# cvYouTian/Dedark-YOLO

Hardware: AMD Instinct MI355X
Metric: training img/s at 640x640 (higher is better)
Workload: dtype bf16

## Files before the change

### dedark_yolo_amd/csrc/conv_v5.hip

```cpp
#include <stdlib.h>
#include <type_traits>
#include "dy_common.h"
#include "conv_epilogue.h"
#include "../../include/dedark_yolo.h"

namespace v5 {

constexpr int BM = 256, BK = 32;
constexpr int A_BYTES = BM * 64, NSTAGE = 3;
constexpr unsigned B_ROW_OOB = 0x40000000u;

typedef __attribute__((address_space(3))) void* lds_ptr_t;
typedef __attribute__((ext_vector_type(8))) __bf16 bf16x8;

__device__ unsigned long long g_stamps[16];

__device__ inline void stamp(int ablate, int nblk, int i) {
  if ((ablate & 32) && threadIdx.x == 0 && (blockIdx.x == 0 || (int)blockIdx.x == (nblk / 8) * 7)) {
    unsigned long long t;
    asm volatile("s_memtime %0\n\ts_waitcnt lgkmcnt(0)" : "=s"(t)::"memory");
    g_stamps[(blockIdx.x == 0 ? 0 : 8) + i] = t;
  }
}

struct P {
  const char* src;
  const char* w;
  char* dst;
  unsigned src_bytes, w_bytes;
  long src_ld, dst_ld, dst_row, dst_img;
  int Hs, Ws, Cs, Hd, Wd, Cd;
  int stride;
  int KH, KW;
  int dh0, dhs, dw0, dws;
  int kh0, khs, kw0, kws, KWf;
  long w_row;
  const float* scale;
  const float* shift;
  int act;
  double* stats;
  int accumulate;
  long M;
  int a_min;
  int nk;
  int tiles_n, nblk;
  const char* add_src;
  long add_src_ld;
  int ablate;
  int ncls;
  DyParityCls cls[4];
};

__device__ inline int xcd_remap(int bid, int nblk) {
  int q = nblk >> 3, r = nblk & 7, x = bid & 7;
  int base = (x < r) ? x * (q + 1) : r * (q + 1) + (x - r) * q;
  return base + (bid >> 3);
}

__device__ inline long dst_offset(const P& p, long m) {
  if (p.dst_row == 0) return m * p.dst_ld;
  const long HWd = (long)p.Hd * p.Wd;
  const long img = m / HWd;
  const int rem = (int)(m - img * HWd);
  const int oh = rem / p.Wd, ow = rem - oh * p.Wd;
  return img * p.dst_img + (long)oh * p.dst_row + (long)ow * p.dst_ld;
}

template <int BN, typename T, int MB>
__device__ __forceinline__ void epilogue(const P& p, f32x4 (&acc)[MB][4], char* smem, int tid, int lane, int wave, int wm, int wn, long m0,
                                         int n0, int tile_m) {
  constexpr int WN = BN / 64, WM = 4 / WN;
  constexpr int PT = dy_epi::row_pitch<BN>();
  const int cl = lane & 15, g = lane >> 4;
  const bool plain = !p.scale && !p.shift && p.act == DY_ACT_NONE;
#pragma unroll
  for (int j = 0; j < 4; ++j) {
    const int c0 = 64 * wn + 16 * j + 4 * g;
    if (plain) {
#pragma unroll
      for (int i = 0; i < MB; ++i) {
        const int px = 16 * MB * wm + 16 * i + cl;
        uint2 w2 = {dy_epi::pack2<T>(acc[i][j][0], acc[i][j][1]), dy_epi::pack2<T>(acc[i][j][2], acc[i][j][3])};
        *reinterpret_cast<uint2*>(smem + px * PT + c0 * 2) = w2;
      }
    } else {
      float sc[4], sf[4];
#pragma unroll
      for (int e = 0; e < 4; ++e) {
        const int n = n0 + c0 + e;
        const bool nok = n < p.Cd;
        sc[e] = (nok && p.scale) ? p.scale[n] : 1.f;
        sf[e] = (nok && p.shift) ? p.shift[n] : 0.f;
      }
#pragma unroll
      for (int i = 0; i < MB; ++i) {
        const int px = 16 * MB * wm + 16 * i + cl;
        float v[4];
#pragma unroll
        for (int e = 0; e < 4; ++e) {
          float u = acc[i][j][e] * sc[e] + sf[e];
          if (p.act == DY_ACT_SILU) u = u * dy_sigmoid(u);
          else if (p.act == DY_ACT_LEAKY) u = u > 0.f ? u : 0.1f * u;
          v[e] = u;
        }
        uint2 w2 = {dy_epi::pack2<T>(v[0], v[1]), dy_epi::pack2<T>(v[2], v[3])};
        *reinterpret_cast<uint2*>(smem + px * PT + c0 * 2) = w2;
      }
    }
  }
  __syncthreads();
  stamp(DY_ABLATE_OF(p), p.nblk, 3);
  dy_epi::store_rows<BM, BN, 4>(smem, lane, wave, m0, n0, p.M, p.Cd, p.accumulate, reinterpret_cast<T*>(p.dst),
                                [&](long m) { return dst_offset(p, m); }, reinterpret_cast<const T*>(p.add_src), p.add_src_ld);
  stamp(DY_ABLATE_OF(p), p.nblk, 4);
  if (p.stats) {
    __syncthreads();
    float* red = reinterpret_cast<float*>(smem);
#pragma unroll
    for (int j = 0; j < 4; ++j)
#pragma unroll
      for (int e = 0; e < 4; ++e) {
        float s1 = 0.f, s2 = 0.f;
#pragma unroll
        for (int i = 0; i < MB; ++i) {
          const float a = acc[i][j][e];
          s1 += a;
          s2 += a * a;
        }
        s1 = row16_sum(s1);
        s2 = row16_sum(s2);
        if (cl == 0) {
          const int col = 64 * wn + 16 * j + 4 * g + e;
          red[(wm * BN + col) * 2] = s1;
          red[(wm * BN + col) * 2 + 1] = s2;
        }
      }
    __syncthreads();
    if (tid < BN) {
      const int n = n0 + tid;
      if (n < p.Cd) {
        float s1 = 0.f, s2 = 0.f;
#pragma unroll
        for (int w = 0; w < WM; ++w) {
          s1 += red[(w * BN + tid) * 2];
          s2 += red[(w * BN + tid) * 2 + 1];
        }
        double* st = p.stats + (long)(tile_m % DY_STATS_REPLICAS) * 2 * p.Cd;
        atomic_add_f64(st + n, (double)s1);
        atomic_add_f64(st + p.Cd + n, (double)s2);
      }
    }
  }
}

template <int BN, typename T = bf16_t, bool SLIM = false>
__global__ __launch_bounds__(256, SLIM ? 4 : 2) void conv_kernel(const P pk) {
  constexpr int WN = BN / 64, WM = 4 / WN, MB = BM / WM / 16, NB = 4, STAGE = A_BYTES + BN * 64, B_LD = BN / 64;
  extern __shared__ __attribute__((aligned(16))) char smem[];
  const int tid = threadIdx.x, lane = tid & 63;
  const int wave = __builtin_amdgcn_readfirstlane(tid >> 6);
  const int wm = wave / WN, wn = wave % WN;
  P p = pk;
  int bid;
  if (pk.ncls > 1) {
    const int x = blockIdx.x & 7, i = (int)blockIdx.x >> 3;
    int c = 0;
#pragma unroll
    for (int k = 1; k < 4; ++k)
      if (k < pk.ncls && i >= pk.cls[k].blk0) c = k;
    const DyParityCls& k = pk.cls[c];
    bid = x * k._r + (i - k.blk0);
    if (bid >= (int)((k.M + BM - 1) / BM) * pk.tiles_n) return;
    p.dst = k.dst; p.M = k.M; p.Hd = k.Hd; p.Wd = k.Wd; p.KH = k.KH; p.KW = k.KW;
    p.dh0 = -k.pad; p.dw0 = -k.pad; p.kh0 = k.kh0; p.kw0 = k.kw0;
    p.nk = k.Ktot / BK;
    p.a_min = -(k.pad * pk.Ws + k.pad) * (int)pk.src_ld * 2;
  } else {
    bid = xcd_remap(blockIdx.x, p.nblk);
  }
  stamp(DY_ABLATE_OF(p), p.nblk, 0);
  const int tile_m = bid / p.tiles_n, tile_n = bid - tile_m * p.tiles_n;
  const long m0 = (long)tile_m * BM;
  const int n0 = tile_n * BN;

  unsigned nrec_a = p.nk > 0 ? p.src_bytes - p.a_min : 0, nrec_b = p.nk > 0 ? p.w_bytes : 0;

  const int lrow = lane >> 2, slot = lane & 3;
  const int chunk = slot ^ ((lane & 32) ? 3 : 0);
  unsigned a_off[4], a_pad[4], b_off[B_LD];
  {
    const DyTileWalk walk(m0, p.Hd, p.Wd);
#pragma unroll
    for (int j = 0; j < 4; ++j) {
      const int r = 16 * (wave + 4 * j) + lrow;
      const bool ok = m0 + r < p.M;
      int img, oh, ow;
      walk.at(r, img, oh, ow);
      const int sh0 = oh * p.stride, sw0 = ow * p.stride;
      a_off[j] = (unsigned)((((long)img * p.Hs + sh0) * p.Ws + sw0) * p.src_ld * 2 + chunk * 16);
      unsigned wb = 0, mk = 0;
      for (int tw = 0; tw < p.KW; ++tw) {
        const int sw = sw0 + p.dw0 + p.dws * tw;
        if (sw >= 0 && sw < p.Ws) wb |= 1u << tw;
      }
      for (int th = 0; th < p.KH; ++th) {
        const int sh = sh0 + p.dh0 + p.dhs * th;
        if (ok && sh >= 0 && sh < p.Hs) mk |= wb << (th * p.KW);
      }
      if (DY_ABLATE_OF(p) & 2) mk = 0;
      else if (DY_ABLATE_OF(p) & 1) mk &= 1u;
      a_pad[j] = __builtin_amdgcn_alignbit(~mk, ~mk, 1);
    }
#pragma unroll
    for (int j = 0; j < B_LD; ++j) {
      const int n = n0 + 16 * (wave + 4 * j) + lrow;
      b_off[j] = (n < p.Cd && !(DY_ABLATE_OF(p) & 4)) ? (unsigned)((long)n * p.w_row * 2 + chunk * 16) : B_ROW_OOB;
    }
  }
  const int ntaps = p.KH * p.KW;
  int vtap_a, vtap_b;
  {
    const int t = lane < ntaps ? lane : 0;
    const int th = t / p.KW, tw = t - th * p.KW;
    vtap_a = ((p.dh0 + p.dhs * th) * p.Ws + p.dw0 + p.dws * tw) * (int)p.src_ld * 2 - p.a_min;
    vtap_b = (int)((((long)((p.kh0 + p.khs * th) * p.KWf + p.kw0 + p.kws * tw)) * p.Cs) * 2);
  }
  int sk = 0, s_tap = 0, s_ci2 = 0;
  int a_koff = __builtin_amdgcn_readlane(vtap_a, 0), b_koff = __builtin_amdgcn_readlane(vtap_b, 0);
  auto advance = [&]() {
    ++sk;
    const bool wrap = s_tap + 1 == ntaps;
    s_tap = wrap ? 0 : s_tap + 1;
    s_ci2 += wrap ? 2 * BK : 0;
    a_koff = __builtin_amdgcn_readlane(vtap_a, s_tap) + s_ci2;
    b_koff = __builtin_amdgcn_readlane(vtap_b, s_tap) + s_ci2;
    const int rot = wrap ? (33 - ntaps) & 31 : 1;
#pragma unroll
    for (int j = 0; j < 4; ++j) a_pad[j] = __builtin_amdgcn_alignbit(a_pad[j], a_pad[j], rot);
    if (sk >= p.nk) { nrec_a = 0; nrec_b = 0; a_koff = 0; b_koff = 0; }
  };
  auto issue = [&](int base) {
    const __amdgpu_buffer_rsrc_t rs_a = __builtin_amdgcn_make_buffer_rsrc((void*)(p.src + p.a_min), 0, nrec_a, 0x00020000);
    const __amdgpu_buffer_rsrc_t rs_b = __builtin_amdgcn_make_buffer_rsrc((void*)p.w, 0, nrec_b, 0x00020000);
#pragma unroll
    for (int j = 0; j < 4; ++j) {
      if ((DY_ABLATE_OF(p) & 64) && s_tap) continue;
      const unsigned v = (a_pad[j] & 0x80000000u) | a_off[j];
      __builtin_amdgcn_raw_ptr_buffer_load_lds(rs_a, (lds_ptr_t)(smem + base + (wave + 4 * j) * 1024), 16, (int)v, a_koff, 0, 0);
    }
#pragma unroll
    for (int j = 0; j < B_LD; ++j)
      __builtin_amdgcn_raw_ptr_buffer_load_lds(rs_b, (lds_ptr_t)(smem + base + A_BYTES + (wave + 4 * j) * 1024), 16, (int)b_off[j], b_koff, 0,
                                               0);
  };

  const int fr = lane & 15, fq = lane >> 4;
  const int sw = (fq ^ ((fr & 8) ? 3 : 0)) * 16;
  const int a_rd = (16 * MB * wm + fr) * 64 + sw;
  const int b_rd = A_BYTES + (64 * wn + fr) * 64 + sw;

  f32x4 acc[MB][NB];
#pragma unroll
  for (int i = 0; i < MB; ++i)
#pragma unroll
    for (int j = 0; j < 4; ++j) acc[i][j] = f32x4{0.f, 0.f, 0.f, 0.f};

  auto compute = [&](int base, auto mid) {
    u32x4 bfr[NB], afr[MB];
    if (DY_ABLATE_OF(p) & 16) {
#pragma unroll
      for (int j = 0; j < 4; ++j) bfr[j] = u32x4{0x3f803f80u + (unsigned)base, 0x3f803f80u, 0x3f803f80u, 0x3f803f80u};
#pragma unroll
      for (int i = 0; i < MB; ++i) afr[i] = u32x4{0x3f803f80u, 0x3f803f80u + (unsigned)lane, 0x3f803f80u, 0x3f803f80u};
    } else {
#pragma unroll
      for (int j = 0; j < 4; ++j) bfr[j] = *reinterpret_cast<const u32x4*>(smem + base + b_rd + 1024 * j);
#pragma unroll
      for (int i = 0; i < MB; ++i) afr[i] = *reinterpret_cast<const u32x4*>(smem + base + a_rd + 1024 * i);
    }
    if (DY_ABLATE_OF(p) & 8) {
#pragma unroll
      for (int i = 0; i < MB; ++i) acc[i][0][0] += __builtin_bit_cast(float, afr[i][0] ^ bfr[i & 3][1]);
      mid();
      return;
    }
    __builtin_amdgcn_s_setprio(1);
#pragma unroll
    for (int i = 0; i < MB; ++i) {
#pragma unroll
      for (int j = 0; j < NB; ++j)
        acc[i][j] = mfma_16x16x32<T>(bfr[j], afr[i], acc[i][j]);
      if (i == 0) mid();
    }
    __builtin_amdgcn_s_setprio(0);
  };
  auto nothing = []() {};
  auto walk = [&]() { advance(); };
  stamp(DY_ABLATE_OF(p), p.nblk, 1);
  if constexpr (BN >= 128) {
    issue(0);
    advance();
    issue(STAGE);
    advance();
    int cur = 0, fill = 2 * STAGE;
    for (int kt = 0; kt < p.nk; ++kt) {
      if ((DY_ABLATE_OF(p) & 64) || kt + 1 >= p.nk) asm volatile("s_waitcnt vmcnt(0)" ::: "memory");
      else
      asm volatile("s_waitcnt vmcnt(%0)" ::"n"(4 + B_LD) : "memory");
      __builtin_amdgcn_s_barrier();
      __builtin_amdgcn_sched_barrier(0);
      if (sk < p.nk) issue(fill);
      __builtin_amdgcn_sched_barrier(0);
      compute(cur, walk);
      __builtin_amdgcn_sched_barrier(0);
      cur = cur == 2 * STAGE ? 0 : cur + STAGE;
      fill = fill == 2 * STAGE ? 0 : fill + STAGE;
    }
  } else if constexpr (SLIM) {
    issue(0);
    advance();
    int cur = 0;
    for (int kt = 0; kt < p.nk; ++kt) {
      asm volatile("s_waitcnt vmcnt(0)" ::: "memory");
      __builtin_amdgcn_s_barrier();
      __builtin_amdgcn_sched_barrier(0);
      if (sk < p.nk) issue(cur ? 0 : STAGE);
      __builtin_amdgcn_sched_barrier(0);
      compute(cur, walk);
      __builtin_amdgcn_sched_barrier(0);
      cur = cur ? 0 : STAGE;
    }
  } else {
    issue(0);
    advance();
    issue(STAGE);
    advance();
    int cur = 0;
    for (int kt = 0; kt < p.nk; kt += 2) {
      asm volatile("s_waitcnt vmcnt(0)" ::: "memory");
      __builtin_amdgcn_s_barrier();
      __builtin_amdgcn_sched_barrier(0);
      const int nxt = cur ^ (2 * STAGE);
      if (sk < p.nk) {
        issue(nxt);
        advance();
        issue(nxt + STAGE);
      } else {
        advance();
      }
      __builtin_amdgcn_sched_barrier(0);
      compute(cur, walk);
      compute(cur + STAGE, nothing);
      __builtin_amdgcn_sched_barrier(0);
      cur = nxt;
    }
  }
  asm volatile("s_waitcnt vmcnt(0)" ::: "memory");
  __builtin_amdgcn_s_barrier();
  stamp(DY_ABLATE_OF(p), p.nblk, 2);

  epilogue<BN, T, MB>(p, acc, smem, tid, lane, wave, wm, wn, m0, n0, tile_m);
#ifdef DY_DIAG
  asm volatile("s_waitcnt vmcnt(0)" ::: "memory");
#endif
  stamp(DY_ABLATE_OF(p), p.nblk, 5);
}

constexpr int BAND_BYTES = 17 * 1024;

template <int BN, typename T = bf16_t, int NBAND_ = (BN == 64 ? 3 : 2)>
__global__ __launch_bounds__(256, (BN == 64 && NBAND_ == 2) ? 3 : 2) void band_kernel(const P p) {
  constexpr int WN = BN / 64, WM = 4 / WN, MB = BM / WM / 16, B_LD = BN / 64, B_BYTES = BN * 64;
  constexpr int NBAND = NBAND_, DB = 3 * (NBAND - 1), NBBUF = DB + 1;
  constexpr int OFF_B = NBAND * BAND_BYTES, OFF_ZERO = OFF_B + NBBUF * B_BYTES;
  constexpr int N0 = (DB - 1) * B_LD + 5 * (NBAND - 2), N1 = (DB - 1) * B_LD + 5 * (NBAND - 1);
  extern __shared__ __attribute__((aligned(16))) char smem[];
  const int tid = threadIdx.x, lane = tid & 63;
  const int wave = __builtin_amdgcn_readfirstlane(tid >> 6);
  const int wm = wave / WN, wn = wave % WN;
  const int bid = xcd_remap(blockIdx.x, p.nblk);
  stamp(DY_ABLATE_OF(p), p.nblk, 0);
  const int tile_m = bid / p.tiles_n, tile_n = bid - tile_m * p.tiles_n;
  const long m0 = (long)tile_m * BM;
  const int n0 = tile_n * BN;

  if (tid < 16) reinterpret_cast<unsigned*>(smem + OFF_ZERO)[tid] = 0u;

  const int lrow = lane >> 2, slot = lane & 3;
  const int chunk = slot ^ ((lane & 16) ? 2 : 0);
  const bool tail_lane = (lane >> 4) == wave;
  unsigned a_off[5], b_off[B_LD];
#pragma unroll
  for (int j = 0; j < 5; ++j) {
    const int brow = j < 4 ? 16 * (wave + 4 * j) + lrow : 256 + lrow;
    a_off[j] = (unsigned)((m0 - 1 + brow) * p.src_ld * 2 + chunk * 16);
  }
#pragma unroll
  for (int j = 0; j < B_LD; ++j) {
    const int n = n0 + 16 * (wave + 4 * j) + lrow;
    b_off[j] = n < p.Cd ? (unsigned)((long)n * p.w_row * 2 + chunk * 16) : B_ROW_OOB;
  }
  const int ng = p.nk / 3;
  int ga_n = 0, ga_th = 0, ga_ci = 0;
  auto issue_band = [&](int base) {
    const bool live = ga_n < ng && !(DY_ABLATE_OF(p) & 2);
    const unsigned koff = (unsigned)((p.dh0 + p.dhs * ga_th) * p.Ws * (int)p.src_ld * 2 + ga_ci * 2);
    const __amdgpu_buffer_rsrc_t rs = __builtin_amdgcn_make_buffer_rsrc((void*)p.src, 0, live ? p.src_bytes : 0u, 0x00020000);
#pragma unroll
    for (int j = 0; j < 4; ++j)
      __builtin_amdgcn_raw_ptr_buffer_load_lds(rs, (lds_ptr_t)(smem + base + (wave + 4 * j) * 1024), 16, (int)(a_off[j] + koff), 0, 0, 0);
    if (tail_lane)
      __builtin_amdgcn_raw_ptr_buffer_load_lds(rs, (lds_ptr_t)(smem + base + 16 * 1024), 16, (int)(a_off[4] + koff), 0, 0, 0);
    ++ga_n;
    if (++ga_th == 3) { ga_th = 0; ga_ci += BK; }
  };
  int kb = 0, kb_tp = 0, kb_ci = 0;
  auto issue_b = [&](int base) {
    const bool live = kb < p.nk && !(DY_ABLATE_OF(p) & 4);
    const int koff = live ? (int)(((long)kb_tp * p.Cs + kb_ci) * 2) : 0;
    const __amdgpu_buffer_rsrc_t rs = __builtin_amdgcn_make_buffer_rsrc((void*)p.w, 0, live ? p.w_bytes : 0u, 0x00020000);
#pragma unroll
    for (int j = 0; j < B_LD; ++j)
      __builtin_amdgcn_raw_ptr_buffer_load_lds(rs, (lds_ptr_t)(smem + base + (wave + 4 * j) * 1024), 16, (int)b_off[j], koff, 0, 0);
    ++kb;
    if (++kb_tp == 9) { kb_tp = 0; kb_ci += BK; }
  };

  const int fr = lane & 15, fq = lane >> 4;
  const int r0 = 16 * MB * wm + fr;
  int a_rd[3];
#pragma unroll
  for (int tw = 0; tw < 3; ++tw) {
    const int brow = r0 + 1 + p.dw0 + p.dws * tw;
    a_rd[tw] = brow * 64 + ((fq ^ ((brow & 4) ? 2 : 0)) * 16);
  }
  const int b_rd = (64 * wn + fr) * 64 + ((fq ^ ((fr & 4) ? 2 : 0)) * 16);
  unsigned tm[3] = {0u, 0u, 0u};
  {
    const long m = m0 + r0;
    int img, h, w;
    DyTileWalk(m0, p.Hd, p.Wd).at(r0, img, h, w);
#pragma unroll
    for (int i = 0; i < MB; ++i) {
      const bool ok = m + 16 * i < p.M;
#pragma unroll
      for (int th = 0; th < 3; ++th) {
        const bool hv = (unsigned)(h + p.dh0 + p.dhs * th) < (unsigned)p.Hs;
#pragma unroll
        for (int tw = 0; tw < 3; ++tw) {
          const bool wv = (unsigned)(w + p.dw0 + p.dws * tw) < (unsigned)p.Ws;
          if (ok && hv && wv) tm[th] |= 1u << (8 * tw + i);
        }
      }
      w += 16;
      if (w >= p.Wd) {
        w -= p.Wd;
        if (++h == p.Hd) h = 0;
      }
    }
  }

  f32x4 acc[MB][4];
#pragma unroll
  for (int i = 0; i < MB; ++i)
#pragma unroll
    for (int j = 0; j < 4; ++j) acc[i][j] = f32x4{0.f, 0.f, 0.f, 0.f};

  auto compute = [&](int band_base, int b_base, unsigned bits, int ard) {
    u32x4 bfr[4], afr[MB];
    const int av = band_base + ard;
    if (DY_ABLATE_OF(p) & 16) {
#pragma unroll
      for (int j = 0; j < 4; ++j) bfr[j] = u32x4{0x3f803f80u + (unsigned)b_base, 0x3f803f80u, 0x3f803f80u, 0x3f803f80u};
#pragma unroll
      for (int i = 0; i < MB; ++i) afr[i] = u32x4{0x3f803f80u, 0x3f803f80u + (bits & 1u), 0x3f803f80u, 0x3f803f80u};
    } else {
#pragma unroll
      for (int j = 0; j < 4; ++j) bfr[j] = *reinterpret_cast<const u32x4*>(smem + b_base + b_rd + 1024 * j);
#pragma unroll
      for (int i = 0; i < MB; ++i) {
        const int sel = ((bits >> i) & 1u) ? av : OFF_ZERO - 1024 * i;
        afr[i] = *reinterpret_cast<const u32x4*>(smem + sel + 1024 * i);
      }
    }
    if (DY_ABLATE_OF(p) & 8) {
#pragma unroll
      for (int i = 0; i < MB; ++i) acc[i][0][0] += __builtin_bit_cast(float, afr[i][0] ^ bfr[i & 3][1]);
      return;
    }
    __builtin_amdgcn_s_setprio(1);
#pragma unroll
    for (int i = 0; i < MB; ++i)
#pragma unroll
      for (int j = 0; j < 4; ++j) acc[i][j] = mfma_16x16x32<T>(bfr[j], afr[i], acc[i][j]);
    __builtin_amdgcn_s_setprio(0);
  };
  stamp(DY_ABLATE_OF(p), p.nblk, 1);

  int band_fill = 0, b_fill = 0;
#pragma unroll
  for (int s = 0; s < DB; ++s) {
    if (s % 3 == 0) {
      issue_band(band_fill);
      band_fill += BAND_BYTES;
    }
    issue_b(OFF_B + b_fill);
    b_fill += B_BYTES;
  }
  int band_cur = 0, b_cur = 0, th = 0;
  auto next_b = [&]() {
    b_cur = b_cur == DB * B_BYTES ? 0 : b_cur + B_BYTES;
    b_fill = b_fill == DB * B_BYTES ? 0 : b_fill + B_BYTES;
  };
  auto group = [&](auto tailc) {
    constexpr bool tail = decltype(tailc)::value;
    const unsigned tmc = th == 0 ? tm[0] : (th == 1 ? tm[1] : tm[2]);
    asm volatile("s_waitcnt vmcnt(%0)" ::"n"(N0) : "memory");
    __builtin_amdgcn_s_barrier();
    __builtin_amdgcn_sched_barrier(0);
    if constexpr (!tail) {
      issue_band(band_fill);
      issue_b(OFF_B + b_fill);
    }
    __builtin_amdgcn_sched_barrier(0);
    compute(band_cur, OFF_B + b_cur, tmc, a_rd[0]);
    __builtin_amdgcn_sched_barrier(0);
    next_b();
    asm volatile("s_waitcnt vmcnt(%0)" ::"n"(tail ? B_LD : N1) : "memory");
    __builtin_amdgcn_s_barrier();
    __builtin_amdgcn_sched_barrier(0);
    if constexpr (!tail) issue_b(OFF_B + b_fill);
    __builtin_amdgcn_sched_barrier(0);
    compute(band_cur, OFF_B + b_cur, tmc >> 8, a_rd[1]);
    __builtin_amdgcn_sched_barrier(0);
    next_b();
    asm volatile("s_waitcnt vmcnt(%0)" ::"n"(tail ? 0 : N1) : "memory");
    __builtin_amdgcn_s_barrier();
    __builtin_amdgcn_sched_barrier(0);
    if constexpr (!tail) issue_b(OFF_B + b_fill);
    __builtin_amdgcn_sched_barrier(0);
    compute(band_cur, OFF_B + b_cur, tmc >> 16, a_rd[2]);
    __builtin_amdgcn_sched_barrier(0);
    next_b();
    band_cur = band_cur == (NBAND - 1) * BAND_BYTES ? 0 : band_cur + BAND_BYTES;
    band_fill = band_fill == (NBAND - 1) * BAND_BYTES ? 0 : band_fill + BAND_BYTES;
    th = th == 2 ? 0 : th + 1;
  };
  constexpr bool peel = NBAND == 2;
  for (int g = 0; g < ng - (peel ? 1 : 0); ++g) group(std::false_type{});
  if (peel) group(std::true_type{});
  asm volatile("s_waitcnt vmcnt(0)" ::: "memory");
  __builtin_amdgcn_s_barrier();
  stamp(DY_ABLATE_OF(p), p.nblk, 2);
  epilogue<BN, T, MB>(p, acc, smem, tid, lane, wave, wm, wn, m0, n0, tile_m);
#ifdef DY_DIAG
  asm volatile("s_waitcnt vmcnt(0)" ::: "memory");
#endif
  stamp(DY_ABLATE_OF(p), p.nblk, 5);
}


}

extern "C" int dy_debug_conv5_stamps(unsigned long long* out) {
  return hipMemcpyFromSymbol(out, HIP_SYMBOL(v5::g_stamps), sizeof(unsigned long long) * 16) == hipSuccess ? 0 : 1;
}

bool dy_conv_v5_eligible(const dy_conv_desc* d, int mode) {
  static const bool off = dy_env("DY_NO_CONV_V5") != nullptr;
  if (off || (d->dtype != DY_BF16 && d->dtype != DY_F16)) return false;
  if (!(d->Cs % 32 == 0 && d->KH * d->KW <= 25)) return false;
  if (mode == 1 && d->stride != 1) return false;
  if ((d->src_ld * 2) % 16 != 0 || (d->dst_ld * 2) % 16 != 0 || ((uintptr_t)d->dst) % 16 != 0) return false;
  const long M = (long)d->N * d->Hd * d->Wd;
  const long src_bytes = (((long)d->N * d->Hs * d->Ws - 1) * d->src_ld + d->Cs) * 2;
  const long w_row = d->KHf > 0 ? (long)d->KHf * d->KWf * d->Cs : (long)d->KH * d->KW * d->Cs;
  const long w_bytes = (long)d->Cd * w_row * 2;
  const long halo = ((long)d->KH * d->dil * d->Ws + (long)d->KW * d->dil) * d->src_ld * 2;
  if (!(src_bytes + halo <= 0x7fffffffL && w_bytes <= 0x3fffffffL && M < (1L << 31))) return false;
  const long tiles_m = (M + 255) / 256;
  const long tn = (d->Cd + 127) / 128;
  if (d->Cd >= 96 && tn * 128 * 4 <= (long)d->Cd * 5 && tiles_m * tn >= 256) return true;
  return d->Cd >= 48 && d->Cd <= 64 && tiles_m >= 256;
}

static int v5_launch(const dy_conv_desc* d, int mode, void* stream, const dy_conv_desc* classes, int ncls);

int dy_conv_v5_launch(const dy_conv_desc* d, int mode, void* stream) { return v5_launch(d, mode, stream, nullptr, 0); }

bool dy_conv_v5_classes_eligible(const dy_conv_desc* c, int ncls) {
  static const bool off = dy_env("DY_NO_CONV_V5") != nullptr || (dy_env("DY_V5_CLASSES") && atoi(dy_env("DY_V5_CLASSES")) == 0);
  if (off || ncls < 2 || ncls > 4) return false;
  const dy_conv_desc* d = &c[0];
  if (d->dtype != DY_BF16 && d->dtype != DY_F16) return false;
  if (!(d->Cs % 32 == 0 && d->KHf > 0 && d->KHf * d->KWf <= 25 && d->stride == 1)) return false;
  const long src_bytes = (((long)d->N * d->Hs * d->Ws - 1) * d->src_ld + d->Cs) * 2;
  const long w_bytes = (long)d->Cd * d->KHf * d->KWf * d->Cs * 2;
  const long halo = ((long)d->KHf * d->Ws + d->KWf) * d->src_ld * 2;
  if (!(src_bytes + halo <= 0x7fffffffL && w_bytes <= 0x3fffffffL)) return false;
  const long tn = (d->Cd + 127) / 128;
  const bool wide = d->Cd >= 96 && tn * 128 * 4 <= (long)d->Cd * 5, narrow = d->Cd >= 48 && d->Cd <= 64;
  if (!wide && !narrow) return false;
  long tiles = 0;
  for (int i = 0; i < ncls; ++i) {
    const dy_conv_desc& q = c[i];
    if (q.src != d->src || q.w != d->w || q.Cs != d->Cs || q.Cd != d->Cd || q.dtype != d->dtype || q.stride != 1 || q.dil != 1 || q.KHf != d->KHf ||
        q.KWf != d->KWf || q.kh_step != d->kh_step || q.kw_step != d->kw_step || q.dst_ld != d->dst_ld || q.dst_row_stride != d->dst_row_stride ||
        q.dst_img_stride != d->dst_img_stride || q.src_ld != d->src_ld || q.accumulate != d->accumulate || q.scale || q.shift || q.stats ||
        q.act != DY_ACT_NONE)
      return false;
    if ((q.dst_ld * 2) % 16 != 0 || ((uintptr_t)q.dst) % 16 != 0 || (q.src_ld * 2) % 16 != 0) return false;
    if ((long)q.N * q.Hd * q.Wd >= (1L << 31)) return false;
    tiles += (((long)q.N * q.Hd * q.Wd + 255) / 256) * (wide ? tn : 1);
  }
  return tiles >= 256;
}

int dy_conv_v5_launch_classes(const dy_conv_desc* c, int ncls, void* stream) { return v5_launch(&c[0], 0, stream, c, ncls); }

static int v5_launch(const dy_conv_desc* d, int mode, void* stream, const dy_conv_desc* classes, int ncls) {
  v5::P p;
  p.src = (const char*)d->src; p.w = (const char*)d->w; p.dst = (char*)d->dst;
  p.src_ld = d->src_ld; p.dst_ld = d->dst_ld;
  p.src_bytes = (unsigned)((((long)d->N * d->Hs * d->Ws - 1) * d->src_ld + d->Cs) * 2);
  p.Hs = d->Hs; p.Ws = d->Ws; p.Cs = d->Cs; p.Hd = d->Hd; p.Wd = d->Wd; p.Cd = d->Cd;
  p.KH = d->KH; p.KW = d->KW;
  if (mode == 0) {
    p.stride = d->stride; p.dh0 = -d->pad; p.dhs = d->dil; p.dw0 = -d->pad; p.dws = d->dil;
  } else {
    p.stride = 1; p.dh0 = d->pad; p.dhs = -d->dil; p.dw0 = d->pad; p.dws = -d->dil;
  }
  if (d->KHf > 0) {
    p.kh0 = d->kh0; p.khs = d->kh_step; p.kw0 = d->kw0; p.kws = d->kw_step; p.KWf = d->KWf;
    p.w_row = (long)d->KHf * d->KWf * d->Cs;
  } else {
    p.kh0 = 0; p.khs = 1; p.kw0 = 0; p.kws = 1; p.KWf = d->KW;
    p.w_row = (long)d->KH * d->KW * d->Cs;
  }
  p.w_bytes = (unsigned)((long)d->Cd * p.w_row * 2);
  {
    const int dh_lo = p.dhs < 0 ? p.dh0 + p.dhs * (p.KH - 1) : p.dh0, dw_lo = p.dws < 0 ? p.dw0 + p.dws * (p.KW - 1) : p.dw0;
    const long lo = ((long)dh_lo * p.Ws + dw_lo) * p.src_ld * 2;
    p.a_min = lo < 0 ? (int)lo : 0;
  }
  p.scale = d->scale; p.shift = d->shift; p.act = d->act; p.stats = d->stats; p.accumulate = d->accumulate;
  if ((long)d->N * d->Hd * d->Wd * d->Cd * 2 > (128L << 20)) p.accumulate |= 2;
  p.M = (long)d->N * d->Hd * d->Wd;
  p.add_src = mode == 1 ? (const char*)d->add_src : nullptr; p.add_src_ld = d->add_src_ld;
  p.nk = d->KH * d->KW * d->Cs / v5::BK;
  static const int ablate = dy_env("DY_ABLATE") ? atoi(dy_env("DY_ABLATE")) : 0;
  p.ablate = ablate;
  p.dst_row = d->dst_row_stride;
  p.dst_img = d->dst_img_stride ? d->dst_img_stride : (long)d->Hd * d->dst_row_stride;
  const int bn = d->Cd <= 64 ? 64 : 128;
  p.tiles_n = dy_cdiv(d->Cd, bn);
  p.nblk = dy_cdiv(p.M, v5::BM) * p.tiles_n;
  p.ncls = 0;
  if (ncls > 1) {
    DY_CHECK(ncls <= 4 && mode == 0, "conv_v5: at most 4 forward-style classes");
    p.ncls = ncls;
    int slot = 0;
    for (int c = 0; c < ncls; ++c) {
      const dy_conv_desc& q = classes[c];
      DyParityCls& k = p.cls[c];
      k.dst = (char*)q.dst; k.M = (long)q.N * q.Hd * q.Wd; k.Hd = q.Hd; k.Wd = q.Wd; k.KH = q.KH; k.KW = q.KW; k.pad = q.pad;
      k.kh0 = q.kh0; k.kw0 = q.kw0; k.Ktot = q.KH * q.KW * q.Cs;
      const int tiles = (int)dy_cdiv(k.M, (long)v5::BM) * p.tiles_n;
      k.blk0 = slot;
      k._r = dy_cdiv(tiles, 8);
      slot += k._r;
    }
    p.nblk = 8 * slot;
  }
  constexpr int RING128 = v5::NSTAGE * (v5::A_BYTES + 128 * 64), EPI128 = dy_epi::row_image_bytes<v5::BM, 128>();
  constexpr int RING64 = 4 * (v5::A_BYTES + 64 * 64), EPI64 = dy_epi::row_image_bytes<v5::BM, 64>();
  constexpr int SH128 = RING128 > EPI128 ? RING128 : EPI128, SH64 = RING64 > EPI64 ? RING64 : EPI64;
  constexpr int RING64S = 2 * (v5::A_BYTES + 64 * 64), SH64S = RING64S > EPI64 ? RING64S : EPI64;
  static_assert(4 * SH64S <= 160 * 1024, "four blocks per CU");
  static const bool slim64 = !(dy_env("DY_CONV64_SLIM") && atoi(dy_env("DY_CONV64_SLIM")) == 0);
  constexpr int BAND128 = 2 * v5::BAND_BYTES + 4 * 128 * 64 + 64, BAND64 = 3 * v5::BAND_BYTES + 7 * 64 * 64 + 64;
  constexpr int SB128 = BAND128 > EPI128 ? BAND128 : EPI128, SB64 = BAND64 > EPI64 ? BAND64 : EPI64;
  constexpr int BAND64S = 2 * v5::BAND_BYTES + 4 * 64 * 64 + 64, SB64S = BAND64S > EPI64 ? BAND64S : EPI64;
  static_assert(3 * SB64S <= 160 * 1024, "three blocks per CU");
  static const int band64_nband = dy_env("DY_BAND64_NBAND") ? atoi(dy_env("DY_BAND64_NBAND")) : 2;
  static_assert(2 * SH128 <= 160 * 1024 && 2 * SH64 <= 160 * 1024 && 2 * SB128 <= 160 * 1024 && 2 * SB64 <= 160 * 1024, "two blocks per CU");
  static const bool no_band = dy_env("DY_NO_CONV_BAND") != nullptr;
  const bool band = ncls <= 1 && !no_band && d->KH == 3 && d->KW == 3 && d->stride == 1 && d->pad == 1 && d->dil == 1 && d->KHf <= 0 && d->Hs == d->Hd &&
                    d->Ws == d->Wd && d->Ws >= 16;
  static bool configured = false;
  if (!configured) {
    hipError_t e = hipFuncSetAttribute(reinterpret_cast<const void*>(&v5::conv_kernel<128, bf16_t>), hipFuncAttributeMaxDynamicSharedMemorySize, SH128);
    if (e == hipSuccess) e = hipFuncSetAttribute(reinterpret_cast<const void*>(&v5::conv_kernel<64, bf16_t>), hipFuncAttributeMaxDynamicSharedMemorySize, SH64);
    if (e == hipSuccess) e = hipFuncSetAttribute(reinterpret_cast<const void*>(&v5::conv_kernel<128, f16_t>), hipFuncAttributeMaxDynamicSharedMemorySize, SH128);
    if (e == hipSuccess) e = hipFuncSetAttribute(reinterpret_cast<const void*>(&v5::conv_kernel<64, f16_t>), hipFuncAttributeMaxDynamicSharedMemorySize, SH64);
    if (e == hipSuccess) e = hipFuncSetAttribute(reinterpret_cast<const void*>(&v5::conv_kernel<64, bf16_t, true>), hipFuncAttributeMaxDynamicSharedMemorySize, SH64S);
    if (e == hipSuccess) e = hipFuncSetAttribute(reinterpret_cast<const void*>(&v5::conv_kernel<64, f16_t, true>), hipFuncAttributeMaxDynamicSharedMemorySize, SH64S);
    if (e == hipSuccess) e = hipFuncSetAttribute(reinterpret_cast<const void*>(&v5::band_kernel<128, bf16_t>), hipFuncAttributeMaxDynamicSharedMemorySize, SB128);
    if (e == hipSuccess) e = hipFuncSetAttribute(reinterpret_cast<const void*>(&v5::band_kernel<64, bf16_t>), hipFuncAttributeMaxDynamicSharedMemorySize, SB64);
    if (e == hipSuccess) e = hipFuncSetAttribute(reinterpret_cast<const void*>(&v5::band_kernel<128, f16_t>), hipFuncAttributeMaxDynamicSharedMemorySize, SB128);
    if (e == hipSuccess) e = hipFuncSetAttribute(reinterpret_cast<const void*>(&v5::band_kernel<64, f16_t>), hipFuncAttributeMaxDynamicSharedMemorySize, SB64);
    if (e == hipSuccess) e = hipFuncSetAttribute(reinterpret_cast<const void*>(&v5::band_kernel<64, bf16_t, 2>), hipFuncAttributeMaxDynamicSharedMemorySize, SB64S);
    if (e == hipSuccess) e = hipFuncSetAttribute(reinterpret_cast<const void*>(&v5::band_kernel<64, f16_t, 2>), hipFuncAttributeMaxDynamicSharedMemorySize, SB64S);
    if (e != hipSuccess) {
      dy_set_error("conv_v5: hipFuncSetAttribute failed: %s", hipGetErrorString(e));
      return 3;
    }
    configured = true;
  }
  const bool f16 = d->dtype == DY_F16;
  if (band && bn == 128) {
    dy_note_kernel("v5::band_kernel<128>");
    if (f16) v5::band_kernel<128, f16_t><<<p.nblk, 256, SB128, (hipStream_t)stream>>>(p);
    else v5::band_kernel<128, bf16_t><<<p.nblk, 256, SB128, (hipStream_t)stream>>>(p);
  } else if (band && band64_nband == 2) {
    dy_note_kernel("v5::band_kernel<64>");
    if (f16) v5::band_kernel<64, f16_t, 2><<<p.nblk, 256, SB64S, (hipStream_t)stream>>>(p);
    else v5::band_kernel<64, bf16_t, 2><<<p.nblk, 256, SB64S, (hipStream_t)stream>>>(p);
  } else if (band) {
    dy_note_kernel("v5::band_kernel<64>");
    if (f16) v5::band_kernel<64, f16_t><<<p.nblk, 256, SB64, (hipStream_t)stream>>>(p);
    else v5::band_kernel<64, bf16_t><<<p.nblk, 256, SB64, (hipStream_t)stream>>>(p);
  } else if (bn == 128) {
    dy_note_kernel("v5::conv_kernel<128>");
    if (f16) v5::conv_kernel<128, f16_t><<<p.nblk, 256, SH128, (hipStream_t)stream>>>(p);
    else v5::conv_kernel<128, bf16_t><<<p.nblk, 256, SH128, (hipStream_t)stream>>>(p);
  } else if (slim64) {
    dy_note_kernel("v5::conv_kernel<64>");
    if (f16) v5::conv_kernel<64, f16_t, true><<<p.nblk, 256, SH64S, (hipStream_t)stream>>>(p);
    else v5::conv_kernel<64, bf16_t, true><<<p.nblk, 256, SH64S, (hipStream_t)stream>>>(p);
  } else {
    dy_note_kernel("v5::conv_kernel<64>");
    if (f16) v5::conv_kernel<64, f16_t><<<p.nblk, 256, SH64, (hipStream_t)stream>>>(p);
    else v5::conv_kernel<64, bf16_t><<<p.nblk, 256, SH64, (hipStream_t)stream>>>(p);
  }
  DY_LAUNCH_CHECK();
  return 0;
}
```

Measured before the change: 1031.

## Add persistent band-resident 3x3 conv kernel with register-held weights for Cs=64

Adds a persistent kernel for 3x3 stride-1 convolutions with 64 input and at most 64 output channels and no fused epilogue. Each block walks a contiguous run of 128-row tiles, keeps the input rows in a ring buffer in LDS, and holds all weights in registers. The store of each tile's output overlaps the prefetch of the next tile's rows. It avoids reloading the halo rows and weights for every tile, at the cost of one block per CU, heavy register use and a serial walk within each block.

```diff
diff --git a/dedark_yolo_amd/csrc/conv_v5.hip b/dedark_yolo_amd/csrc/conv_v5.hip
--- a/dedark_yolo_amd/csrc/conv_v5.hip
+++ b/dedark_yolo_amd/csrc/conv_v5.hip
@@ -1,5 +1,6 @@
 #include <stdlib.h>
 #include <type_traits>
+#include <utility>
 #include "dy_common.h"
 #include "conv_epilogue.h"
 #include "../../include/dedark_yolo.h"
@@ -44,6 +45,7 @@
   int a_min;
   int nk;
   int tiles_n, nblk;
+  int res_tpb;
   const char* add_src;
   long add_src_ld;
   int ablate;
@@ -557,6 +559,223 @@
   asm volatile("s_waitcnt vmcnt(0)" ::: "memory");
 #endif
   stamp(DY_ABLATE_OF(p), p.nblk, 5);
+}
+
+template <typename F, int... S>
+__device__ __forceinline__ void for_each_step(F&& f, std::integer_sequence<int, S...>) {
+  (f(std::integral_constant<int, S>{}), ...);
+}
+
+constexpr int RES_TM = 128, RES_R = 608, RES_G = RES_R / 16, RES_RB = RES_R * 64;
+constexpr int RES_PS = RES_RB + 64;
+constexpr int RES_ZERO = RES_RB, RES_SMEM = 2 * RES_PS;
+constexpr int RES_MAX_W = 175;
+
+template <typename T, int KIND>
+__global__ __launch_bounds__(256, 1) void band_resident_kernel(const P p) {
+  constexpr bool STATS = KIND == 0;
+  extern __shared__ __attribute__((aligned(16))) char smem[];
+  const int tid = threadIdx.x, lane = tid & 63;
+  const int wave = __builtin_amdgcn_readfirstlane(tid >> 6);
+  const int wm = wave >> 1, wn = wave & 1;
+  const int fr = lane & 15, fq = lane >> 4;
+  const int bid = xcd_remap(blockIdx.x, p.nblk);
+  const long tiles = (p.M + RES_TM - 1) / RES_TM;
+  const long t0 = (long)bid * p.res_tpb;
+  const int nt = (int)(tiles - t0 < p.res_tpb ? tiles - t0 : p.res_tpb);
+  const int W = p.Ws;
+  const int halo = (W + 1 + 15) & ~15, hg = halo >> 4;
+  long m0 = t0 * RES_TM;
+  const long b0 = m0 - halo;
+
+  if (tid < 32) reinterpret_cast<unsigned*>(smem + (tid >> 4) * RES_PS + RES_ZERO)[tid & 15] = 0u;
+
+  const unsigned lane_off = (unsigned)((lane >> 2) * (int)p.src_ld * 2 + (((lane & 3) ^ ((lane & 16) ? 2 : 0)) * 16));
+  const __amdgpu_buffer_rsrc_t rs = __builtin_amdgcn_make_buffer_rsrc((void*)p.src, 0, p.src_bytes, 0x00020000);
+  auto issue = [&](int ug, int rg, int pl) {
+    const unsigned base = (unsigned)((b0 + 16L * ug) * p.src_ld * 2 + pl * 64);
+    __builtin_amdgcn_raw_ptr_buffer_load_lds(rs, (lds_ptr_t)(smem + pl * RES_PS + rg * 1024), 16, (int)(lane_off + base), 0, 0, 0);
+  };
+  const int g0 = RES_TM / 16 + 2 * hg;
+  for (int idx = wave; idx < 2 * g0; idx += 4) issue(idx >> 1, idx >> 1, idx & 1);
+  int fill_u = g0, fill_r = g0;
+
+  u32x4 wr[18][2];
+#pragma unroll
+  for (int s = 0; s < 18; ++s)
+#pragma unroll
+    for (int j = 0; j < 2; ++j) {
+      const int n = 32 * wn + 8 * (fr >> 2) + 4 * j + (fr & 3);
+      const int c = s / 9, t = s - 9 * c;
+      const u32x4 v = *reinterpret_cast<const u32x4*>(p.w + ((long)(n < p.Cd ? n : 0) * p.w_row + t * 64 + 32 * c) * 2 + fq * 16);
+      wr[s][j] = n < p.Cd ? v : u32x4{0u, 0u, 0u, 0u};
+    }
+
+  unsigned xlo = (unsigned)((halo - W - 1 + 64 * wm + fr) * 64 + fq * 16);
+  int hs, ws;
+  {
+    int img;
+    DyTileWalk(m0, p.Hd, p.Wd).at(64 * wm + fr, img, hs, ws);
+  }
+  auto step16 = [&](int& h, int& w) {
+    w += 16;
+    if (w >= p.Wd) {
+      w -= p.Wd;
+      if (++h == p.Hd) h = 0;
+    }
+  };
+
+  f32x4 acc[4][2];
+  float s1[STATS ? 8 : 1], s2[STATS ? 8 : 1];
+  if (STATS) {
+#pragma unroll
+    for (int e = 0; e < 8; ++e) s1[e] = s2[e] = 0.f;
+  }
+  const bool nt_store = p.accumulate & 2;
+  T* const dst = reinterpret_cast<T*>(p.dst);
+  const int n8 = 32 * wn + 8 * fq;
+
+  for (int q = 0; q <= nt; ++q) {
+    asm volatile("s_waitcnt vmcnt(0)" ::: "memory");
+    __builtin_amdgcn_s_barrier();
+    __builtin_amdgcn_sched_barrier(0);
+    if (q + 1 < nt) {
+#pragma unroll
+      for (int j = 0; j < 4; ++j) {
+        const int idx = wave + 4 * j, g = idx >> 1;
+        int rg = fill_r + g;
+        rg = rg >= RES_G ? rg - RES_G : rg;
+        issue(fill_u + g, rg, idx & 1);
+      }
+      fill_u += 8;
+      fill_r = fill_r + 8 >= RES_G ? fill_r + 8 - RES_G : fill_r + 8;
+    }
+    __builtin_amdgcn_sched_barrier(0);
+    if (q > 0) {
+      const long mp = m0 - RES_TM + 64 * wm + fr;
+      const bool nok = n8 < p.Cd;
+      u32x4 v[4];
+#pragma unroll
+      for (int i = 0; i < 4; ++i)
+        v[i] = u32x4{dy_epi::pack2<T>(acc[i][0][0], acc[i][0][1]), dy_epi::pack2<T>(acc[i][0][2], acc[i][0][3]),
+                     dy_epi::pack2<T>(acc[i][1][0], acc[i][1][1]), dy_epi::pack2<T>(acc[i][1][2], acc[i][1][3])};
+      if constexpr (KIND == 2) {
+        const T* const add = reinterpret_cast<const T*>(p.add_src);
+        const bool accum = p.accumulate & 1;
+        u32x4 old[4], av[4];
+#pragma unroll
+        for (int i = 0; i < 4; ++i) {
+          const long m = mp + 16 * i;
+          const bool ok = nok && m < p.M;
+          old[i] = (ok && accum) ? *reinterpret_cast<const u32x4*>(dst + m * p.dst_ld + n8) : u32x4{0u, 0u, 0u, 0u};
+          av[i] = (ok && add) ? *reinterpret_cast<const u32x4*>(add + m * p.add_src_ld + n8) : u32x4{0u, 0u, 0u, 0u};
+        }
+#pragma unroll
+        for (int i = 0; i < 4; ++i) {
+          float x[8], y[8];
+          ldvec<T>(reinterpret_cast<const T*>(&v[i]), y);
+          if (accum) {
+            ldvec<T>(reinterpret_cast<const T*>(&old[i]), x);
+#pragma unroll
+            for (int e = 0; e < 8; ++e) y[e] += x[e];
+          }
+          if (add) {
+            ldvec<T>(reinterpret_cast<const T*>(&av[i]), x);
+#pragma unroll
+            for (int e = 0; e < 8; ++e) y[e] += x[e];
+          }
+          stvec<T>(reinterpret_cast<T*>(&v[i]), y);
+        }
+      }
+#pragma unroll
+      for (int i = 0; i < 4; ++i) {
+        const long m = mp + 16 * i;
+        if (nok && m < p.M) {
+          T* o = dst + m * p.dst_ld + n8;
+          if (nt_store) asm volatile("global_store_dwordx4 %0, %1, off nt" ::"v"(o), "v"(v[i]) : "memory");
+          else *reinterpret_cast<u32x4*>(o) = v[i];
+        }
+      }
+    }
+    if (q == nt) break;
+
+    unsigned mk[4];
+    {
+      int h = hs, w = ws;
+      const long m = m0 + 64 * wm + fr;
+#pragma unroll
+      for (int i = 0; i < 4; ++i) {
+        unsigned hb = 0u, wb = 0u;
+#pragma unroll
+        for (int t = 0; t < 3; ++t) {
+          if ((unsigned)(h + p.dh0 + p.dhs * t) < (unsigned)p.Hs) hb |= 1u << (3 * t);
+          if ((unsigned)(w + p.dw0 + p.dws * t) < (unsigned)p.Ws) wb |= 1u << t;
+        }
+        mk[i] = m + 16 * i < p.M ? hb * wb : 0u;
+        step16(h, w);
+      }
+#pragma unroll
+      for (int i = 0; i < 4; ++i) step16(h, w);
+      hs = h;
+      ws = w;
+    }
+#pragma unroll
+    for (int i = 0; i < 4; ++i)
+#pragma unroll
+      for (int j = 0; j < 2; ++j) acc[i][j] = f32x4{0.f, 0.f, 0.f, 0.f};
+
+    u32x4 afr[3][4];
+    auto fetch = [&](auto sc, u32x4 (&fr4)[4]) {
+      constexpr int s = decltype(sc)::value, c = s / 9, t = s - 9 * c, th = t / 3, tw = t - 3 * th;
+      const unsigned toff = (unsigned)(((p.dh0 + p.dhs * th + 1) * W + p.dw0 + p.dws * tw + 1) * 64);
+#pragma unroll
+      for (int i = 0; i < 4; ++i) {
+        unsigned x = xlo + toff + 1024u * i;
+        x = x < x - RES_RB ? x : x - RES_RB;
+        x ^= (x >> 3) & 32u;
+        const unsigned in = (unsigned)((int)(mk[i] << (31 - t)) >> 31);
+        x = (x & in) | ((unsigned)RES_ZERO & ~in);
+        fr4[i] = *reinterpret_cast<const u32x4*>(smem + x + c * RES_PS);
+      }
+    };
+    auto step = [&](auto sc) {
+      constexpr int s = decltype(sc)::value;
+      if constexpr (s + 2 < 18) fetch(std::integral_constant<int, (s + 2 < 18 ? s + 2 : 0)>{}, afr[(s + 2) % 3]);
+#pragma unroll
+      for (int i = 0; i < 4; ++i)
+#pragma unroll
+        for (int j = 0; j < 2; ++j) acc[i][j] = mfma_16x16x32<T>(wr[s][j], afr[s % 3][i], acc[i][j]);
+      __builtin_amdgcn_sched_barrier(0);
+    };
+    fetch(std::integral_constant<int, 0>{}, afr[0]);
+    fetch(std::integral_constant<int, 1>{}, afr[1]);
+    __builtin_amdgcn_sched_barrier(0);
+    for_each_step(step, std::make_integer_sequence<int, 18>{});
+    if (STATS) {
+#pragma unroll
+      for (int i = 0; i < 4; ++i)
+#pragma unroll
+        for (int e = 0; e < 8; ++e) {
+          const float a = acc[i][e >> 2][e & 3];
+          s1[e] += a;
+          s2[e] += a * a;
+        }
+    }
+    m0 += RES_TM;
+    xlo += RES_TM * 64;
+    xlo = xlo < xlo - RES_RB ? xlo : xlo - RES_RB;
+  }
+  if (STATS) {
+    double* st = p.stats + (long)(bid % DY_STATS_REPLICAS) * 2 * p.Cd;
+#pragma unroll
+    for (int e = 0; e < 8; ++e) {
+      const float a = row16_sum(s1[e]), b = row16_sum(s2[e]);
+      if (fr == 0 && n8 + e < p.Cd) {
+        atomic_add_f64(st + n8 + e, (double)a);
+        atomic_add_f64(st + p.Cd + n8 + e, (double)b);
+      }
+    }
+  }
 }
 
 
@@ -656,6 +875,7 @@
   p.tiles_n = dy_cdiv(d->Cd, bn);
   p.nblk = dy_cdiv(p.M, v5::BM) * p.tiles_n;
   p.ncls = 0;
+  p.res_tpb = 0;
   if (ncls > 1) {
     DY_CHECK(ncls <= 4 && mode == 0, "conv_v5: at most 4 forward-style classes");
     p.ncls = ncls;
@@ -683,13 +903,38 @@
   constexpr int BAND64S = 2 * v5::BAND_BYTES + 4 * 64 * 64 + 64, SB64S = BAND64S > EPI64 ? BAND64S : EPI64;
   static_assert(3 * SB64S <= 160 * 1024, "three blocks per CU");
   static const int band64_nband = dy_env("DY_BAND64_NBAND") ? atoi(dy_env("DY_BAND64_NBAND")) : 2;
+  static_assert(v5::RES_SMEM <= 160 * 1024, "resident ring");
   static_assert(2 * SH128 <= 160 * 1024 && 2 * SH64 <= 160 * 1024 && 2 * SB128 <= 160 * 1024 && 2 * SB64 <= 160 * 1024, "two blocks per CU");
   static const bool no_band = dy_env("DY_NO_CONV_BAND") != nullptr;
   const bool band = ncls <= 1 && !no_band && d->KH == 3 && d->KW == 3 && d->stride == 1 && d->pad == 1 && d->dil == 1 && d->KHf <= 0 && d->Hs == d->Hd &&
                     d->Ws == d->Wd && d->Ws >= 16;
+  static const bool no_resident = dy_env("DY_NO_BAND_RESIDENT") != nullptr;
+  bool resident = false;
+  if (band && bn == 64 && !no_resident && d->Cs == 64 && d->Ws <= v5::RES_MAX_W && !d->scale && !d->shift && d->act == DY_ACT_NONE &&
+      d->Cd % 8 == 0 && d->dst_row_stride == 0 && !(d->stats && (d->accumulate || p.add_src))) {
+    static int ncu = 0;
+    if (ncu == 0) {
+      int dev = 0, n = 0;
+      if (hipGetDevice(&dev) != hipSuccess || hipDeviceGetAttribute(&n, hipDeviceAttributeMultiprocessorCount, dev) != hipSuccess || n <= 0) n = 256;
+      ncu = n;
+    }
+    const long tiles = dy_cdiv(p.M, (long)v5::RES_TM);
+    const long tpb = dy_cdiv(tiles, (long)ncu);
+    const long reach = (long)p.src_bytes + (2L * v5::RES_TM + 2 * 176 + 16) * d->src_ld * 2;
+    if (tpb >= 4 && reach <= 0x7fffffffL) {
+      resident = true;
+      p.res_tpb = (int)tpb;
+      p.nblk = (int)dy_cdiv(tiles, tpb);
+    }
+  }
   static bool configured = false;
   if (!configured) {
-    hipError_t e = hipFuncSetAttribute(reinterpret_cast<const void*>(&v5::conv_kernel<128, bf16_t>), hipFuncAttributeMaxDynamicSharedMemorySize, SH128);
+    hipError_t e = hipSuccess;
+    for (const void* fn : {reinterpret_cast<const void*>(&v5::band_resident_kernel<bf16_t, 0>), reinterpret_cast<const void*>(&v5::band_resident_kernel<bf16_t, 1>),
+                           reinterpret_cast<const void*>(&v5::band_resident_kernel<bf16_t, 2>), reinterpret_cast<const void*>(&v5::band_resident_kernel<f16_t, 0>),
+                           reinterpret_cast<const void*>(&v5::band_resident_kernel<f16_t, 1>), reinterpret_cast<const void*>(&v5::band_resident_kernel<f16_t, 2>)})
+      if (e == hipSuccess) e = hipFuncSetAttribute(fn, hipFuncAttributeMaxDynamicSharedMemorySize, v5::RES_SMEM);
+    if (e == hipSuccess) e = hipFuncSetAttribute(reinterpret_cast<const void*>(&v5::conv_kernel<128, bf16_t>), hipFuncAttributeMaxDynamicSharedMemorySize, SH128);
     if (e == hipSuccess) e = hipFuncSetAttribute(reinterpret_cast<const void*>(&v5::conv_kernel<64, bf16_t>), hipFuncAttributeMaxDynamicSharedMemorySize, SH64);
     if (e == hipSuccess) e = hipFuncSetAttribute(reinterpret_cast<const void*>(&v5::conv_kernel<128, f16_t>), hipFuncAttributeMaxDynamicSharedMemorySize, SH128);
     if (e == hipSuccess) e = hipFuncSetAttribute(reinterpret_cast<const void*>(&v5::conv_kernel<64, f16_t>), hipFuncAttributeMaxDynamicSharedMemorySize, SH64);
@@ -708,7 +953,20 @@
     configured = true;
   }
   const bool f16 = d->dtype == DY_F16;
-  if (band && bn == 128) {
+  if (resident) {
+    dy_note_kernel("v5::band_kernel<64>[resident]");
+    const hipStream_t st = (hipStream_t)stream;
+    const int kind = p.stats ? 0 : (((p.accumulate & 1) || p.add_src) ? 2 : 1);
+    if (f16) {
+      if (kind == 0) v5::band_resident_kernel<f16_t, 0><<<p.nblk, 256, v5::RES_SMEM, st>>>(p);
+      else if (kind == 1) v5::band_resident_kernel<f16_t, 1><<<p.nblk, 256, v5::RES_SMEM, st>>>(p);
+      else v5::band_resident_kernel<f16_t, 2><<<p.nblk, 256, v5::RES_SMEM, st>>>(p);
+    } else {
+      if (kind == 0) v5::band_resident_kernel<bf16_t, 0><<<p.nblk, 256, v5::RES_SMEM, st>>>(p);
+      else if (kind == 1) v5::band_resident_kernel<bf16_t, 1><<<p.nblk, 256, v5::RES_SMEM, st>>>(p);
+      else v5::band_resident_kernel<bf16_t, 2><<<p.nblk, 256, v5::RES_SMEM, st>>>(p);
+    }
+  } else if (band && bn == 128) {
     dy_note_kernel("v5::band_kernel<128>");
     if (f16) v5::band_kernel<128, f16_t><<<p.nblk, 256, SB128, (hipStream_t)stream>>>(p);
     else v5::band_kernel<128, bf16_t><<<p.nblk, 256, SB128, (hipStream_t)stream>>>(p);
```

New measurement: 1031, median of 3. Within noise of the previous version (+0.0%).
